# fgcallari/skeres

Hardware: AMD Instinct MI355X
Metric: LM iterations/sec (higher is better)
Workload: dtype f64

## Files before the change

### skeres_amd/csrc/bal_kernels.hip

```cpp
#include <hip/hip_runtime.h>
#include "functors.hpp"
#include "bal_kernels.hpp"

namespace sk {

static constexpr int kBlock = 256;

__device__ __forceinline__ double wave_sum(double v) {
#pragma unroll
  for (int off = 32; off > 0; off >>= 1) v += __shfl_xor(v, off, 64);
  return v;
}

__device__ __forceinline__ int bal_part(const BalDev& d, int i) { return i >= d.cam_b ? 2 : ((i >= d.seg_lo && i < d.cam_a) ? 0 : 1); }
__device__ __forceinline__ int bal_pos(const BalDev& d, int i, int part) { return 9 * (i - (part == 0 ? d.seg_lo : (part == 1 ? d.cam_a : d.cam_b))); }
__device__ __forceinline__ double* bal_block(const BalDev& d, int i, int j, int* ld) {
  const int pj = bal_part(d, j), pi = bal_part(d, i);
  const BalDev::Front& f = d.front[pj];
  const int row = pi == pj ? bal_pos(d, i, pi) : f.border_row[i - d.cam_b];
  *ld = f.ld;
  return f.S + (size_t)row * f.ld + bal_pos(d, j, pj);
}
__device__ __forceinline__ double* bal_rhs(const BalDev& d, int i) {
  const int pi = bal_part(d, i);
// ... 878 lines not shown
}

__global__ __launch_bounds__(256) void tri_pack_kernel(double* S, int ld, double* packed, const int* __restrict__ col0, const long long* __restrict__ off,
                                                       int to_packed) {
  const int kb = blockIdx.y;
  const size_t c0 = (size_t)col0[kb] * 128, width = (size_t)(kb + 1) * 128 - c0;
  double* pk = packed + off[kb];
  const size_t n2 = 128 * width / 2;
  for (size_t i = (size_t)blockIdx.x * 256 + threadIdx.x; i < n2; i += (size_t)gridDim.x * 256) {
    const size_t e = 2 * i, r = e / width, c = e % width;
    double2* a = reinterpret_cast<double2*>(S + ((size_t)kb * 128 + r) * ld + c0 + c);
    double2* b = reinterpret_cast<double2*>(pk + e);
    if (to_packed) *b = *a; else *a = *b;
  }
}

static inline int grid_for(int n, int cap = 2048) {
  int g = (n + kBlock - 1) / kBlock;
  return g < 1 ? 1 : (g > cap ? cap : g);
}

__global__ __launch_bounds__(256) void zero_envelope_kernel(double* S, int ld, const int* col0) {
  const int kb = blockIdx.y;
  const size_t c0 = (size_t)col0[kb] * 128, width = (size_t)(kb + 1) * 128 - c0;
  const size_t n2 = 128 * width / 2;
  for (size_t i = (size_t)blockIdx.x * 256 + threadIdx.x; i < n2; i += (size_t)gridDim.x * 256) {
    const size_t e = 2 * i, r = e / width, c = e % width;
    *reinterpret_cast<double2*>(S + ((size_t)kb * 128 + r) * ld + c0 + c) = make_double2(0.0, 0.0);
  }
}
void launch_zero_envelope(double* S, int ld, const int* col0, int nblk, hipStream_t s) {
  if (nblk > 0) hipLaunchKernelGGL(zero_envelope_kernel, dim3(32, nblk), dim3(256), 0, s, S, ld, col0);
}

int bal_partial_blocks(int N) { return grid_for(N); }
size_t tri_packed_elems(int nblk) { return (size_t)128 * 128 * ((size_t)nblk * (nblk + 1) / 2); }
void launch_tri_pack(double* S, int ld, double* packed, int nblk, const int* col0, const long long* off, bool to_packed, hipStream_t s) {
  if (nblk > 0) hipLaunchKernelGGL(tri_pack_kernel, dim3(64, nblk), dim3(256), 0, s, S, ld, packed, col0, off, to_packed ? 1 : 0);
}

void launch_bal_eval_jac(const BalDev& d, hipStream_t s) {
  if (d.loss_root >= 0) hipLaunchKernelGGL(bal_eval_jac_kernel<true>, dim3(grid_for(d.N)), dim3(kBlock), 0, s, d);
  else hipLaunchKernelGGL(bal_eval_jac_kernel<false>, dim3(grid_for(d.N)), dim3(kBlock), 0, s, d);
}
void launch_bal_eval_cost(const BalDev& d, hipStream_t s) {
  if (d.loss_root >= 0) hipLaunchKernelGGL(bal_eval_cost_kernel<true>, dim3(grid_for(d.N)), dim3(kBlock), 0, s, d);
  else hipLaunchKernelGGL(bal_eval_cost_kernel<false>, dim3(grid_for(d.N)), dim3(kBlock), 0, s, d);
}
int bal_tape_width(const Tape& t) { return t.num_obs_consts > kTapeMaxObs ? 0 : tape_pick_width(t, kBlock); }
template <class K> static void bal_tape_allow_lds(K kernel, size_t bytes) {
  if (bytes > 48 * 1024) (void)hipFuncSetAttribute(reinterpret_cast<const void*>(kernel), hipFuncAttributeMaxDynamicSharedMemorySize, (int)bytes);
}
void launch_bal_eval_jac_tape(const BalDev& d, const TapeDevBuffers& tb, hipStream_t s) {
  const int W = bal_tape_width(tb.host), nobs = tb.host.num_obs_consts;
  const size_t lds = tape_lds_bytes(tb.host, W, kBlock);
  const dim3 g(grid_for(d.N)), b(kBlock);
#define SK_TAPE_JAC(LOSS, WW) { bal_tape_allow_lds(bal_eval_jac_tape_kernel<LOSS, WW>, lds); hipLaunchKernelGGL((bal_eval_jac_tape_kernel<LOSS, WW>), g, b, lds, s, d, tb.view, nobs); }
  if (d.loss_root >= 0) { if (W == 3) SK_TAPE_JAC(true, 3) else if (W == 2) SK_TAPE_JAC(true, 2) else SK_TAPE_JAC(true, 1) }
  else { if (W == 3) SK_TAPE_JAC(false, 3) else if (W == 2) SK_TAPE_JAC(false, 2) else SK_TAPE_JAC(false, 1) }
#undef SK_TAPE_JAC
}
void launch_bal_eval_cost_tape(const BalDev& d, const TapeDevBuffers& tb, hipStream_t s) {
  const size_t lds = tape_lds_bytes(tb.host, 0, kBlock);
  const int nobs = tb.host.num_obs_consts;
  if (d.loss_root >= 0) { bal_tape_allow_lds(bal_eval_cost_tape_kernel<true>, lds); hipLaunchKernelGGL(bal_eval_cost_tape_kernel<true>, dim3(grid_for(d.N)), dim3(kBlock), lds, s, d, tb.view, nobs); }
  else { bal_tape_allow_lds(bal_eval_cost_tape_kernel<false>, lds); hipLaunchKernelGGL(bal_eval_cost_tape_kernel<false>, dim3(grid_for(d.N)), dim3(kBlock), lds, s, d, tb.view, nobs); }
// ... 117 lines not shown
```

### skeres_amd/csrc/bal_kernels.hpp

```cpp
#pragma once
#include <hip/hip_runtime.h>

#include "common.hpp"
#include "loss.hpp"

namespace sk {

constexpr int kLongSegment = 32;
constexpr int kWs = 32;
constexpr int kWu = 28;
struct BalDev {
  int C, P, N;
  int res_size, cam_size, pt_size;
  const int* cam;
  const int* pt;
  const double* obs;
  const int* pt_start;
  const int* cam_start;
  const int* cam_obs;
  int num_segments;
  const int* seg_start;
  const int* seg_row;
  const int* seg_col;
  int num_short_segments, num_long_segments;
// ... 7 lines not shown
  const unsigned char* pseudo;
  const int* kept_home;  const int* kept_global;
  int num_dup;  const int* dup_a;  const int* dup_b;  const int* dup_cam;
  double* xc;  double* xp;
  double* xc_new;  double* xp_new;
  double* scale_c;  double* scale_p;
  double* colsq_c;  double* colsq_p;
  double* gs_c;  double* gs_p;
  double lm_lo, lm_hi, lm_radius;  const double* lm_radius_dev;
  double* step_c;  double* step_p;
  double* y_c;
  double* r;  double* F;  double* E;  double* What;  double* u;
  double* Fcam;  const int* obs_slot;
  double* M;  double* q;
  struct Front { double* S; int ld; int interior; int rhs_row; const int* border_row; };
  Front front[3];
  int seg_lo, cam_a, cam_b;
  const double* y_front[3];
  double* S;  int ld;  int rhs_row;
  double* partial;  int partial_stride;
  int* fail_flag;
  const LossNode* loss_nodes;  int loss_root;  const int* loss_of_obs;
  const unsigned char* is_host;
  int num_host;
  const int* host_obs;
  const double* host_rows;
};
constexpr int kHostRow = 26;
constexpr int kFcam = 20;

int bal_partial_blocks(int N);
int bal_point_blocks(int P);
void launch_zero_envelope(double* S, int ld, const int* col0, int nblk, hipStream_t s);
size_t tri_packed_elems(int nblk);
void launch_tri_pack(double* S, int ld, double* packed, int nblk, const int* col0, const long long* off, bool to_packed, hipStream_t s);
void launch_bal_eval_jac(const BalDev& d, hipStream_t s);
void launch_bal_eval_cost(const BalDev& d, hipStream_t s);
void launch_bal_eval_jac_tape(const BalDev& d, const TapeDevBuffers& tb, hipStream_t s);
void launch_bal_eval_cost_tape(const BalDev& d, const TapeDevBuffers& tb, hipStream_t s);
int launch_bal_host_jac(const BalDev& d, int partial_off, hipStream_t s);
int launch_bal_host_cost(const BalDev& d, int partial_off, hipStream_t s);
void launch_bal_scale_jac(const BalDev& d, hipStream_t s);
void launch_bal_cam_records(const BalDev& d, hipStream_t s);
void launch_bal_reduce(const BalDev& d, hipStream_t s);
void launch_jacobi_scale(const double* colsq, double* scale, int n, hipStream_t s);
void launch_apply_scale_to_reductions(double* colsq, double* gs, const double* scale, int n, hipStream_t s);
void launch_lm_diagonal(const double* colsq, double* D, int n, double lo, double hi, double radius, hipStream_t s);
int launch_grad_max_xnorm(const double* gs, const double* scale, const double* x, int n, double* partial, int stride, hipStream_t s);
void launch_final_reduce(const double* partial, int stride, int count, int K, int maxmask, double* out, hipStream_t s);
void launch_bal_pack_rank_scalars(const double* scal, double* table, int rank, int world, int mode, bool segmented, hipStream_t s);
struct ReduceRows { int n = 0; int row[4] = {0, 0, 0, 0}, count[4] = {0, 0, 0, 0}, is_max[4] = {0, 0, 0, 0}; double* out[4] = {nullptr, nullptr, nullptr, nullptr}; };
void launch_final_reduce_rows(const double* partial, int stride, const ReduceRows& rows, hipStream_t s);
void launch_bal_point_block(const BalDev& d, hipStream_t s);
void launch_bal_kept_points(const BalDev& d, hipStream_t s);
void launch_bal_kept_sums(const BalDev& d, double* buf, int K, bool gather, hipStream_t s);
void launch_bal_obs_precompute(const BalDev& d, hipStream_t s);
void launch_bal_cam_diag(const BalDev& d, hipStream_t s);
void launch_bal_pair(const BalDev& d, hipStream_t s);
void launch_finish_normal_matrix(double* S, int ld, int n, int npad, int rhs_row, const double* D, hipStream_t s);
void launch_bal_finish_S(const BalDev& d, int parts, hipStream_t s);
struct BalFinishRanges { double* S[4] = {nullptr, nullptr, nullptr, nullptr}; int ld[4] = {0, 0, 0, 0}, from[4] = {0, 0, 0, 0}, to[4] = {0, 0, 0, 0}; double value[4] = {0, 0, 0, 0}; };
void launch_bal_finish_all(const BalDev& d, const BalFinishRanges& r, hipStream_t s);
void launch_set_diagonal(double* S, int ld, int from, int to, double value, hipStream_t s);
void launch_bal_backsub(const BalDev& d, double* out, int norm_lo, int norm_hi, int norm_lo2, int norm_hi2, hipStream_t s);

}
// ... 1 lines not shown
```

### skeres_amd/csrc/bal_solver.hip

```cpp
#include <algorithm>
#include <atomic>
#include <map>
#include <thread>
#include <cmath>
#include <limits>
#include <numeric>

#include "bal_kernels.hpp"
#include "bal_plan.hpp"
#include "solver.hpp"

namespace sk {

namespace {

struct CaptureGuard {
  hipStream_t s; bool active; bool* graph_mode;
  CaptureGuard(hipStream_t st, bool on, bool* gm) : s(st), active(on), graph_mode(gm) {}
  void release() { active = false; }
  ~CaptureGuard() {
    if (!active) return;
    hipGraph_t g = nullptr;
    (void)hipStreamEndCapture(s, &g);
    if (g) (void)hipGraphDestroy(g);
// ... 201 lines not shown
  int choose_distribution(const std::vector<int>& opt);
  struct Structure {
    std::vector<int> ocam, opt;
    std::vector<int> band_ocam, band_opt;
    std::vector<int> env_for_model;
    int Creal = 0;
  };
  int init_queues();
  int plan_layout(Structure* st);
  void plan_pack();
  int prepare_pack();
  int shard_or_replicate(const std::vector<int>& opt);
  int cut_camera_sequence(Structure* st);
  void adopt_cuts(const CutPlan& cuts, int Cband, bool multi, Structure* st);
  int upload_structure(const LocalStructure& ls);
  int allocate_fronts(const FrontLayout& lay);
  int bind_device_view(const LocalStructure& ls);
  int agree_with_ranks();
  bool distribution_decided_ = false;
  std::chrono::steady_clock::time_point setup_t0_, stage_last_;
  void stage(const char* what) {
    if (!dev_knobs().debug_setup) return;
    const auto now = std::chrono::steady_clock::now();
    std::fprintf(stderr, "[skeres_amd] set-up: %-40s %8.1f ms (at %.1f ms)\n", what, std::chrono::duration<double, std::milli>(now - stage_last_).count(),
                 std::chrono::duration<double, std::milli>(now - setup_t0_).count());
    stage_last_ = now;
  }
  CholeskyContext chol_ctx_;
  double* h_scal_ = nullptr;
  int partial_stride_ = 0;
  bool zero_by_backsolve_ = false;
  bool need_full_zero_ = false;
  DevBuf<int> b_zero_min_f_[3];
  bool pair_claimed_ = false;
 public:
  ~BalSolver() override {
    if (pair_claimed_) cholesky_release_pair_servers(&chol_ctx_);
    for (hipGraphExec_t g : {g_step_[0], g_step_[1], g_eval_[0], g_eval_[1]}) if (g) (void)hipGraphExecDestroy(g);
    if (h_scal_) (void)hipHostFree(h_scal_);
  }
};

int BalSolver::choose_distribution(const std::vector<int>& opt) {
  const int W = opt_.world;
  distribution_ = SK_DISTRIBUTION_SHARDED;
  if (W <= 1 || opt_.distribution_mode == SK_DISTRIBUTION_SHARDED) return SK_OK;
  if (opt_.distribution_mode != SK_DISTRIBUTION_REPLICATED) {
    const double per_iter = chain_model::shardable_work_s(chain_model::pair_entries(opt, P_total_), (double)opt.size());
    est_saved_s_ = per_iter * (1.0 - 1.0 / W);
    int rc = allreduce(b_pack_.p, packed_elems_);
    if (rc) return rc;
    SK_HIP_TRY(hipStreamSynchronize(stream_));
    const auto t0 = std::chrono::steady_clock::now();
    for (int rep = 0; rep < 2; ++rep) { rc = allreduce(b_pack_.p, packed_elems_); if (rc) return rc; }
    SK_HIP_TRY(hipStreamSynchronize(stream_));
    double mine = std::chrono::duration<double>(std::chrono::steady_clock::now() - t0).count() / 2.0;
    double vals[1] = {mine};
    const int ops[1] = {0};
    SK_HIP_TRY(b_small_.alloc(2 * 9 * (size_t)C_ + 6 * retained_pts_.size() + 64 + 16 * (size_t)W));
    rc = gather_rank_scalars(vals, 1, ops);
    if (rc) return rc;
    est_allreduce_s_ = vals[0] / W;
    collect_allreduce_time(true);
    phase_[5] = 0.0;
    if (est_allreduce_s_ <= est_saved_s_) return SK_OK;
  }
  distribution_ = SK_DISTRIBUTION_REPLICATED;
  opt_.allreduce = nullptr; opt_.world = 1; opt_.rank = 0;
  b_pack_.release();
  return SK_OK;
}

// ... 574 lines not shown
  if (!std::isfinite(cost_)) return SK_ERR_EVALUATION_FAILED;
  return SK_OK;
}

int BalSolver::try_step(double radius, bool* valid, double* mcc, double* new_cost, double* step_norm) {
  bool chain_lost = false;
  int rc = try_step_once(radius, valid, mcc, new_cost, step_norm, &chain_lost);
  if (rc == SK_OK && chain_lost) rc = try_step_once(radius, valid, mcc, new_cost, step_norm, &chain_lost);
  return rc;
}

int BalSolver::try_step_once(double radius, bool* valid, double* mcc, double* new_cost, double* step_norm, bool* chain_lost) {
  hipStream_t s = stream_;
  *chain_lost = false;
  const size_t nc = 9 * (size_t)C_;
  *valid = false;
  SK_HIP_TRY(hipEventRecord(ev_[kEvBegin], s));
  const bool graph = graph_ok();
  const bool replay = graph && g_step_[parity_] != nullptr;
  bool candidate_failed = false;
  if (graph) {
    h_scal_[32] = radius;
    if (!replay && hipStreamBeginCapture(s, hipStreamCaptureModeThreadLocal) != hipSuccess) { (void)hipGetLastError(); graph_mode_ = false; return try_step_once(radius, valid, mcc, new_cost, step_norm, chain_lost); }
  }
  CaptureGuard capture(s, graph && !replay, &graph_mode_);
  if (!replay) {
  d_.lm_lo = opt_.min_lm_diagonal; d_.lm_hi = opt_.max_lm_diagonal; d_.lm_radius = radius; d_.lm_radius_dev = nullptr;
  if (graph) {
    SK_HIP_TRY(hipMemcpyAsync(b_scal_.p + 12, h_scal_ + 32, sizeof(double), hipMemcpyHostToDevice, s));
    d_.lm_radius_dev = b_scal_.p + 12;
  }
  const int bs_resident = opt_.resident_kernels && cholesky_backsolve_resident(npad_ / 128) ? 1 : 0;
  const bool zero_after = zero_by_backsolve_ && bs_resident;
  kt_.begin("memset_S", s);
  for (int f = 0; f < 3; ++f)
    if (fr_[f].nblk > 0) launch_zero_envelope(d_.front[f].S, (int)fr_[f].dim, (zero_by_backsolve_ && !need_full_zero_) ? b_zero_min_f_[f].p : b_zero_col0_f_[f].p, fr_[f].nblk, s);
  kt_.end("memset_S", s);
  need_full_zero_ = !zero_after;
  SK_HIP_TRY(hipMemsetAsync(b_scal_.p + 14, 0, 2 * sizeof(double), s));
  launch_bal_point_block(d_, s);
  launch_bal_kept_points(d_, s);
  launch_bal_obs_precompute(d_, s);
  kt_.begin("bal_cam_diag", s); launch_bal_cam_diag(d_, s); kt_.end("bal_cam_diag", s);
  kt_.begin("bal_pair", s); launch_bal_pair(d_, s); kt_.end("bal_pair", s);
  if (opt_.allreduce && !segmented_) {
    launch_tri_pack(d_.S, npad_, b_pack_.p, npad_ / 128, b_pack_col0_.p, b_pack_off_.p, true, s);
    int rc = allreduce(b_pack_.p, packed_elems_);
    if (rc) return rc;
    launch_tri_pack(d_.S, npad_, b_pack_.p, npad_ / 128, b_pack_col0_.p, b_pack_off_.p, false, s);
  }
  auto finish_root = [&]() {
    launch_bal_finish_S(d_, 4, s);
    launch_set_diagonal(d_.front[2].S, (int)fr_[2].dim, fr_[2].rhs_row, fr_[2].rhs_row + 1, 1e300, s);
    launch_set_diagonal(d_.front[2].S, (int)fr_[2].dim, fr_[2].rhs_row + 1, (int)fr_[2].dim, 1.0, s);
  };
  if (!segmented_) {
    BalFinishRanges r;
    int k = 0;
    for (int f = 0; f < 2; ++f)
      if (fr_[f].nblk > 0 && fr_[f].ncols * 128 > 9 * fr_[f].cams) { r.S[k] = d_.front[f].S; r.ld[k] = (int)fr_[f].dim; r.from[k] = 9 * fr_[f].cams; r.to[k] = fr_[f].ncols * 128; r.value[k] = 1.0; ++k; }
    r.S[k] = d_.front[2].S; r.ld[k] = (int)fr_[2].dim; r.from[k] = fr_[2].rhs_row; r.to[k] = fr_[2].rhs_row + 1; r.value[k] = 1e300; ++k;
    if ((int)fr_[2].dim > fr_[2].rhs_row + 1) { r.S[k] = d_.front[2].S; r.ld[k] = (int)fr_[2].dim; r.from[k] = fr_[2].rhs_row + 1; r.to[k] = (int)fr_[2].dim; r.value[k] = 1.0; ++k; }
    launch_bal_finish_all(d_, r, s);
  } else {
    launch_bal_finish_S(d_, 3, s);
    for (int f = 0; f < 2; ++f)
      if (fr_[f].nblk > 0) launch_set_diagonal(d_.front[f].S, (int)fr_[f].dim, 9 * fr_[f].cams, fr_[f].ncols * 128, 1.0, s);
  }
  if (!graph) SK_HIP_TRY(hipEventRecord(ev_[kEvAssemble], s));
  CholeskyContext* ctx = opt_.lookahead ? &chol_ctx_ : nullptr;
  int* bs_info = bs_resident ? info_p_ : nullptr;
  double* yf[3] = {b_yf_.p + fr_[0].y_off, b_yf_.p + fr_[1].y_off, b_yf_.p + fr_[2].y_off};
  double* wf[3] = {b_wf_.p + fr_[0].y_off, b_wf_.p + fr_[1].y_off, b_wf_.p + fr_[2].y_off};
  const bool prefilled = bs_resident != 0;
  if (prefilled) SK_HIP_TRY(hipMemsetAsync(b_yf_.p, 0xff, (fr_[0].dim + fr_[1].dim + fr_[2].dim) * sizeof(double), s));
  if (segmented_) {
    const FrontView& L = leaf_;
    const FrontHost& R = fr_[2];
    double* Rs = d_.front[2].S;
    double* RLinv = b_Linv_.p + R.linv_off;
    if (L.ncols > 0) {
      cholesky_factor(L.S, L.ld, L.nblk * 128, L.Linv, info_p_, group_, s, ctx, &kt_, L.last, chain_ok(), L.ncols, L.tail_rows, nullptr, L.tail);
      cholesky_border_add(Rs, (long)R.dim, L.S, L.ld, L.ncols, L.nblk - L.ncols, b_leaf_map_.p, s);
    }
    if (replica_) SK_HIP_TRY(hipMemsetAsync(b_pack_.p, 0, packed_elems_ * sizeof(double), s));
    else launch_tri_pack(Rs, (int)R.dim, b_pack_.p, R.nblk, b_pack_col0_.p, b_pack_off_.p, true, s);
    int rc = allreduce(b_pack_.p, packed_elems_);
    if (rc) return rc;
    launch_tri_pack(Rs, (int)R.dim, b_pack_.p, R.nblk, b_pack_col0_.p, b_pack_off_.p, false, s);
    finish_root();
    cholesky_factor(Rs, (long)R.dim, (int)R.dim, RLinv, info_p_, group_, s, ctx, &kt_, R.env(), chain_ok(), -1, 1, nullptr, R.tl());
    cholesky_backsolve(Rs, (long)R.dim, 9 * R.cams, (int)R.dim, R.rhs_row, RLinv, wf[2], yf[2], s, &kt_, R.env(), bs_info, R.tl(), zero_after, bs_resident, prefilled);
    if (L.ncols > 0) {
      cholesky_gather_map(yf[2], b_leaf_gmap_.p, b_ybB_.p, (L.nblk - L.ncols) * 128, s);
      cholesky_backsolve_front(L.S, L.ld, L.nblk, L.ncols, L.rhs_row, L.Linv, b_ybB_.p, wf[0], yf[0], s, L.last, L.spike, L.tail_rows, bs_info, zero_after, L.tail, nullptr, bs_resident, prefilled);
    }
  } else if (dissected_) {
    cholesky_dissected_factor(ds_, info_p_, group_, s, ctx, &chol_ctx_b_, &kt_, &kt_b_, chain_ok());
    cholesky_dissected_backsolve(ds_, 9 * fr_[2].cams, wf[2], yf[2], wf[0], yf[0], wf[1], yf[1], b_ybB_.p, s, &chol_ctx_b_, &kt_, bs_info, zero_after, bs_resident, prefilled);
  } else {
    const FrontHost& R = fr_[2];
    cholesky_factor(d_.front[2].S, (long)R.dim, (int)R.dim, b_Linv_.p, info_p_, group_, s, ctx, &kt_, R.env(), chain_ok(), -1, 1, nullptr, R.tl());
    cholesky_backsolve(d_.front[2].S, (long)R.dim, n_, (int)R.dim, R.rhs_row, b_Linv_.p, wf[2], yf[2], s, &kt_, R.env(), bs_info, R.tl(), zero_after, bs_resident, prefilled);
  }
  if (!graph) SK_HIP_TRY(hipEventRecord(ev_[kEvChol], s));
  {
    int lo = 0, hi = (int)nc, lo2 = 0, hi2 = 0;
    if (segmented_) {
      lo = 9 * my_lo_; hi = 9 * my_hi_;
      if (role_ == 0) { lo2 = 9 * cam_b_; hi2 = (int)nc; }
    }
    launch_bal_backsub(d_, b_scal_.p + 8, lo, hi, lo2, hi2, s);
  }
  if (!graph) SK_HIP_TRY(hipEventRecord(ev_[kEvBacksub], s));
  kt_.begin("bal_eval_cost", s);
  if (tape_mode_) launch_bal_eval_cost_tape(d_, tape_dev_, s); else launch_bal_eval_cost(d_, s);
  kt_.end("bal_eval_cost", s);
  int nb_cost = bal_partial_blocks(N_);
  if (d_.num_host > 0) {
    int rc = host_callbacks(d_.xc_new, false, &candidate_failed);
    if (rc) return rc;
    nb_cost += launch_bal_host_cost(d_, nb_cost, s);
  }
  launch_final_reduce(b_partial_.p, partial_stride_, nb_cost, 2, 0, b_scal_.p, s);
  if (!graph) SK_HIP_TRY(hipEventRecord(ev_[kEvCost], s));
  SK_HIP_TRY(hipMemcpyAsync(h_scal_, b_scal_.p, 16 * sizeof(double), hipMemcpyDeviceToHost, s));
  }
  const bool dev_gather = rank_table_on_device(4) && !graph;
  if (dev_gather) { int rc = enqueue_rank_table(1, 4); if (rc) return rc; }
  if (graph) {
    if (!replay) { capture.release(); int rc = finish_capture(s, &g_step_[parity_]); if (rc) return rc; if (!graph_mode_) return try_step_once(radius, valid, mcc, new_cost, step_norm, chain_lost); }
    SK_HIP_TRY(hipGraphLaunch(g_step_[parity_], s));
    SK_HIP_TRY(hipEventRecord(ev_[kEvCost], s));
  }
  SK_HIP_TRY(hipStreamSynchronize(s));
  float ms = 0.f;
  if (graph) {
    if (hipEventElapsedTime(&ms, ev_[kEvBegin], ev_[kEvCost]) == hipSuccess) phase_[2] += 1e-3 * ms;
  } else {
    if (hipEventElapsedTime(&ms, ev_[kEvBegin], ev_[kEvAssemble]) == hipSuccess) phase_[1] += 1e-3 * ms;
    if (hipEventElapsedTime(&ms, ev_[kEvAssemble], ev_[kEvChol]) == hipSuccess) phase_[2] += 1e-3 * ms;
    if (hipEventElapsedTime(&ms, ev_[kEvChol], ev_[kEvBacksub]) == hipSuccess) phase_[3] += 1e-3 * ms;
    if (hipEventElapsedTime(&ms, ev_[kEvBacksub], ev_[kEvCost]) == hipSuccess) phase_[4] += 1e-3 * ms;
  }
  int fail = 0, info = 0;
  std::memcpy(&fail, h_scal_ + 14, sizeof(int)); std::memcpy(&info, h_scal_ + 15, sizeof(int));
  if (info != 0) need_full_zero_ = true;
  if (cholesky_note_info(opt_.lookahead ? &chol_ctx_ : nullptr, info) && !opt_.allreduce) {
    if (graph_mode_) {
      for (hipGraphExec_t* g : {&g_step_[0], &g_step_[1], &g_eval_[0], &g_eval_[1]}) if (*g) { (void)hipGraphExecDestroy(*g); *g = nullptr; }
      graph_mode_ = false;
    }
    *chain_lost = true;
    return SK_OK;
  }
  double loc[4] = {h_scal_[0], h_scal_[1], h_scal_[9] + (segmented_ ? h_scal_[8] : 0.0), (double)(fail | info)};
  const int ops4[4] = {0, 0, 0, 1};
  int rc = dev_gather ? fold_rank_table(loc, 4, ops4) : gather_rank_scalars(loc, 4, ops4);
  if (rc) return rc;
  if (opt_.allreduce && loc[3] >= 2.0) cholesky_disable_chain(&chol_ctx_);
  const double step_sq = (segmented_ ? 0.0 : h_scal_[8]) + loc[2];
  if (loc[3] != 0.0 || !std::isfinite(step_sq) || !std::isfinite(loc[1])) return SK_OK;
  *valid = true;
  *mcc = -loc[1];
  *new_cost = candidate_failed ? std::numeric_limits<double>::max() : 0.5 * loc[0];
  *step_norm = std::sqrt(step_sq);
  return SK_OK;
}
// ... 90 lines not shown
```

### skeres_amd/csrc/capi.hip

```cpp
#include <cmath>
#include <cstdlib>
#include <new>

#include "bal_kernels.hpp"
#include "dense_kernels.hpp"
#include "dense_rows_kernels.hpp"
#include "solver.hpp"

using namespace sk;

struct sk_ptrvec { std::vector<double*> v; };
struct sk_loss_function { LossFunction l; };
struct sk_cost_function { CostFunction c; };
struct sk_problem { Problem p; };
struct sk_local_parameterization { LocalParameterization p; };
struct sk_options { Options o; };
struct sk_summary { Summary s; };
struct sk_solver { std::unique_ptr<SolverBase> impl; };

static std::string g_program_name;

#define SK_GUARD_BEGIN try {
#define SK_GUARD_END(ret)                                                   \
  } catch (const std::bad_alloc&) { set_error("out of host memory"); return ret; } \
// ... 14 lines not shown
  }
  const int root = (int)loss_nodes.size() - 1;
  loss_root_of.emplace(std::move(key), root);
  has_loss = true;
  return root;
}
}

namespace sk { int rotation_apply(int op, int row_major, int jet_dim, const double* in, int n, double* out); }

namespace sk {
const DevKnobs& dev_knobs() {
  static const DevKnobs knobs = [] {
    DevKnobs k;
    auto num = [](const char* name, int def) { const char* e = getenv(name); return e ? atoi(e) : def; };
    k.chain_server = num("SK_CHOL_CHAIN_SERVER", 1);
    k.bs_resident = num("SK_BS_RESIDENT", 1);
    k.chain_stamps = getenv("SK_CHAIN_STAMPS");
    k.bs_stamps = getenv("SK_BS_STAMPS");
    if (const char* e = getenv("SK_DEBUG")) {
      const std::string topics = std::string(",") + e + ",";
      k.debug_queues = topics.find(",queues,") != std::string::npos;
      k.debug_envelope = topics.find(",envelope,") != std::string::npos;
      k.debug_segments = topics.find(",segments,") != std::string::npos;
      k.debug_setup = topics.find(",setup,") != std::string::npos;
      k.debug_chain_abort = topics.find(",chain_abort,") != std::string::npos;
    }
    k.queue_shift = num("SK_QUEUE_SHIFT", 0);
    k.chain_queues = num("SK_CHAIN_QUEUES", -1);
    k.pair_max_trailing = num("SK_CHAIN_PAIR_MAX_TRAILING", 0);
    k.dissect_at = num("SK_DISSECT_AT", -1);
    k.schedule_plain = num("SK_SCHEDULE_PLAIN", 0);
    k.chain_xcd_local = num("SK_CHAIN_XCD_LOCAL", 0);
    if (const char* e = getenv("SK_BS_PAIR")) k.bs_pair = atoi(e);
    if (const char* e = getenv("SK_BS_SPREAD")) k.bs_spread = atoi(e);
    if (const char* e = getenv("SK_CHAIN_EARLY_SERVER")) k.chain_early_server = atoi(e);
    if (const char* e = getenv("SK_BULK_RESERVE")) {
      k.bulk_reserve = atoi(e);
      const char* c = strchr(e, ',');
      k.bulk_reserve_early = c ? atoi(c + 1) : k.bulk_reserve;
    }
    return k;
  }();
  return knobs;
}
}

extern "C" {

const char* sk_version(void) { return "skeres_amd 0.1 (gfx950)"; }
const char* sk_last_error(void) { return get_error(); }
void sk_init_logging(const char* name) { g_program_name = name ? name : ""; }
int sk_device_count(void) { int n = 0; if (hipGetDeviceCount(&n) != hipSuccess) return 0; return n; }

double* sk_array_new(int n) { if (n < 0) return nullptr; return static_cast<double*>(std::calloc((size_t)(n > 0 ? n : 1), sizeof(double))); }
void sk_array_free(double* a) { std::free(a); }
double sk_array_getitem(const double* a, int i) { return a[i]; }
void sk_array_setitem(double* a, int i, double v) { a[i] = v; }
double* sk_array_slice(double* buffer, int start) { return &buffer[start]; }
void sk_array_copy_in(double* dst, const double* src, int n) { if (n > 0) std::memcpy(dst, src, (size_t)n * sizeof(double)); }
void sk_array_copy_out(const double* src, double* dst, int n) { if (n > 0) std::memcpy(dst, src, (size_t)n * sizeof(double)); }

int sk_matrix_is_null(double* const* m) { return m == nullptr; }
double* sk_matrix_row(double* const* m, int i) { return m[i]; }

sk_ptrvec* sk_ptrvec_new(void) { return new (std::nothrow) sk_ptrvec(); }
// ... 800 lines not shown
  std::memcpy(&FA[((size_t)nA * 128 + msep) * dA], b, (size_t)ra * sizeof(double));
  for (int t1 = 0; t1 < nt; ++t1)
    for (int t2 = 0; t2 <= t1; ++t2) FB[(size_t)t1 * dB + t2] = A[(size_t)(n - 1 - t2) * n + (n - 1 - t1)];
  for (int i = nt; i < nB * 128; ++i) FB[(size_t)i * dB + i] = 1.0;
  for (int k = 0; k < msep; ++k)
    for (int t = 0; t < nt; ++t) FB[((size_t)nB * 128 + k) * dB + t] = A[(size_t)(n - 1 - t) * n + (ra + msep - 1 - k)];
  for (int t = 0; t < nt; ++t) FB[((size_t)nB * 128 + msep) * dB + t] = b[n - 1 - t];
  for (int i = 0; i < msep; ++i) std::memcpy(&FR[(size_t)i * dR], A + (size_t)(ra + i) * n + ra, (size_t)(i + 1) * sizeof(double));
  std::memcpy(&FR[(size_t)msep * dR], b + ra, (size_t)msep * sizeof(double));
  FR[(size_t)msep * dR + msep] = 1e300;
  for (size_t j = (size_t)msep + 1; j < dR; ++j) FR[j * dR + j] = 1.0;
  std::vector<int> mapB(dR, -1);
  for (int k = 0; k < msep; ++k) mapB[k] = msep - 1 - k;
  mapB[msep] = msep;
  const std::vector<int> lastA = host_block_envelope(FA, dA, nA + E), lastB = host_block_envelope(FB, dB, nB + E);
  DevBuf<double> dFA, dFB, dFR, dLinv, dw, dy; DevBuf<int> dinfo, dmap;
  hipStream_t s = nullptr;
  SK_HIP_TRY(dFA.upload(FA, s)); SK_HIP_TRY(dFB.upload(FB, s)); SK_HIP_TRY(dFR.upload(FR, s)); SK_HIP_TRY(dmap.upload(mapB, s));
  SK_HIP_TRY(dLinv.alloc((size_t)(nA + nB + E) * 128 * 128)); SK_HIP_TRY(dLinv.zero(s));
  SK_HIP_TRY(dw.alloc(dA + dB + 2 * dR)); SK_HIP_TRY(dy.alloc(dA + dB + dR)); SK_HIP_TRY(dy.zero(s)); SK_HIP_TRY(dinfo.alloc(1)); SK_HIP_TRY(dinfo.zero(s));
  SK_HIP_TRY(cholesky_init());
  CholeskyContext ctx, ctxB;
  const bool la = ctx.init() == hipSuccess;
  if (!la) (void)hipGetLastError();
  SK_HIP_TRY(hipStreamCreateWithFlags(&s, hipStreamNonBlocking));
  SK_HIP_TRY(hipDeviceSynchronize());
  if (la) cholesky_prepare(&ctx, s);
  const bool side = la && ctxB.init_secondary(ctx) == hipSuccess;
  if (la && !side) (void)hipGetLastError();
  DissectedSystem d;
  d.A.S = dFA.p; d.A.ld = (long)dA; d.A.nblk = nA + E; d.A.ncols = nA; d.A.last = lastA.data(); d.A.Linv = dLinv.p; d.A.rhs_row = nA * 128 + msep;
  d.B.S = dFB.p; d.B.ld = (long)dB; d.B.nblk = nB + E; d.B.ncols = nB; d.B.last = lastB.data(); d.B.Linv = dLinv.p + (size_t)nA * 128 * 128; d.B.rhs_row = nB * 128 + msep;
  d.R.S = dFR.p; d.R.ld = (long)dR; d.R.nblk = E; d.R.ncols = E; d.R.last = nullptr; d.R.Linv = dLinv.p + (size_t)(nA + nB) * 128 * 128; d.R.rhs_row = msep;
  d.border_blocks = E; d.mapB = dmap.p;
  const bool chain = automatic_plan != 0 && la && ctx.server != nullptr;
  cholesky_dissected_factor(d, dinfo.p, group, s, la ? &ctx : nullptr, side ? &ctxB : nullptr, nullptr, nullptr, chain);
  double *wA = dw.p, *wB = dw.p + dA, *wR = dw.p + dA + dB, *ybB = dw.p + dA + dB + dR;
  double *yA = dy.p, *yB = dy.p + dA, *yR = dy.p + dA + dB;
  cholesky_dissected_backsolve(d, msep, wR, yR, wA, yA, wB, yB, ybB, s, side ? &ctxB : nullptr, nullptr, dinfo.p);
  SK_HIP_TRY(hipStreamSynchronize(s));
  SK_HIP_TRY(hipStreamDestroy(s));
  int info = 0;
  SK_HIP_TRY(hipMemcpy(&info, dinfo.p, sizeof(int), hipMemcpyDeviceToHost));
  if (info == 2) { (void)cholesky_note_info(&ctx, info); set_error("the resident panel chain timed out"); return SK_ERR_HIP; }
  if (info) { set_error("matrix is not positive definite"); return SK_ERR_EVALUATION_FAILED; }
  std::vector<double> y(dA + dB + dR);
  SK_HIP_TRY(hipMemcpy(y.data(), dy.p, y.size() * sizeof(double), hipMemcpyDeviceToHost));
  for (int i = 0; i < ra; ++i) x[i] = y[i];
  for (int t = 0; t < nt; ++t) x[n - 1 - t] = y[dA + t];
  for (int k = 0; k < msep; ++k) x[ra + k] = y[dA + dB + k];
  return SK_OK;
  SK_GUARD_END(SK_ERR_INVALID_ARGUMENT)
}

int sk_cholesky_solve_segments(int n, const double* A, const double* b, double* x, int num_segments, const int* cuts, int group, int automatic_plan) {
  SK_GUARD_BEGIN
  const int R = num_segments;
  if (n <= 0 || !A || !b || !x || R < 2 || !cuts) { set_error("invalid argument"); return SK_ERR_INVALID_ARGUMENT; }
  if (sk_device_count() <= 0) { set_error("no HIP device available: libskeres_amd has no CPU fallback"); return SK_ERR_NO_DEVICE; }
  std::vector<int> sb(R + 1, 0), se(R + 1, 0);
  sb[R] = n;
  for (int k = 1; k < R; ++k) { sb[k] = cuts[2 * (k - 1)]; se[k] = cuts[2 * (k - 1) + 1]; }
  for (int k = 1; k <= R; ++k)
    if (sb[k] < se[k - 1] || (k < R && (se[k] < sb[k] || se[k] > n))) { set_error("invalid cuts"); return SK_ERR_INVALID_ARGUMENT; }
  for (int k = 1; k < R; ++k)
    for (int i = se[k]; i < n; ++i)
      for (int j = 0; j < sb[k]; ++j)
// ... 107 lines not shown
```

### skeres_amd/csrc/chol_kernels.hip

```cpp
#include <hip/hip_runtime.h>
#include <algorithm>
#include <atomic>
#include <chrono>
#include <hip/hip_ext.h>
#include <math.h>
#include <stdlib.h>
#include <string.h>
#include <memory>
#include "chol_kernels.hpp"
#include "device_table.hpp"

namespace sk {

typedef double d4 __attribute__((ext_vector_type(4)));

constexpr int gemm_lds_doubles(int kBKT, int kTM, int kTN) { return 2 * (kTM + kTN) * (kBKT + 2); }
#define SK_GEMM_LDS(kBKT, kTM, kTN) __shared__ __attribute__((aligned(16))) double sh[gemm_lds_doubles(kBKT, kTM, kTN)];
template <int kMode, int kShape, int kBKT, int kPF, int kTM, int kTN>
__device__ __forceinline__ void gemm_nt_f64_body(double* shp, double* C, long ldc, const double* A, long lda, const double* B, long ldb, int K,
                                                 int tiles_m, int skip, int main_t = 0x7fffffff, int jump_t = 0, int main_n = 0x7fffffff,
                                                 int jump_n = 0, int block_id = -1, int* first_column_done = nullptr, int count_cols = 1,
                                                 int* diag_done = nullptr) {
  constexpr int mode = kMode;
  constexpr int kLdT = kBKT + 2;
// ... 2295 lines not shown
      env.tail[c] = (unsigned short)(tail ? std::min(std::max(tail[c], 0), nblk - 1) : nblk - tail_rows);
    }
    if (!prefilled) (void)hipMemsetAsync(y, 0xff, sizeof(double) * (size_t)ni, s);
    const bool spread = zero_after && dev_knobs().bs_spread != 0;
    const int janitors = zero_after ? bs_janitors(ncols) : 0;
    hipLaunchKernelGGL(bs_resident_kernel, dim3(spread ? 8 * ncols : ncols + janitors), dim3(1024), 0, s, Linv, S, ld, (const double*)(S + (long)rhs_row * ld), ni, y, nblk, env, info, ncols, yb,
                       spread ? -1 : janitors, yb_map);
    return;
  }
  hipLaunchKernelGGL(copy_row_kernel, dim3((ni + 255) / 256), dim3(256), 0, s, S + (long)rhs_row * ld, w, ni, ni);
  std::vector<int> first(nblk, 0);
  int c0 = 0;
  if (last)
    for (int kb = 0; kb < nblk - 1; ++kb) {
      while (c0 < kb && last[c0] < kb) ++c0;
      first[kb] = c0;
    }
  const int bfirst = first[ncols < nblk - 1 ? ncols : nblk - 1];
  const int bcol0 = (spike || tail) ? 0 : std::min(bfirst, ncols) * 128;
  if (ni > bcol0)
    hipLaunchKernelGGL(bs_border_kernel, dim3((ni - bcol0 + 63) / 64), dim3(1024), 0, s, S + (long)ncols * 128 * ld, ld, m, yb, w, bcol0, ni);
  for (int kb = ncols - 1; kb >= 0; --kb) {
    const int nc = kb * 128, col0 = first[kb] * 128;
    const int grid = nc > col0 ? (nc - col0 + 63) / 64 : 1;
    hipLaunchKernelGGL(bs_step_kernel, dim3(grid), dim3(1024), 0, s, Linv + (long)kb * 128 * 128, S + (long)kb * 128 * ld, ld, w, y, kb, col0, nc);
  }
}

static void fork_join_events(CholeskyContext* c) {
  if (!c->fork_ev) (void)hipEventCreateWithFlags(&c->fork_ev, g_event_flags);
  if (!c->join_ev) (void)hipEventCreateWithFlags(&c->join_ev, g_event_flags);
}

void cholesky_dissected_factor(const DissectedSystem& d, int* info, int group, hipStream_t s, CholeskyContext* ctxA, CholeskyContext* ctxB,
                               KernelTimer* kt, KernelTimer* ktB, bool allow_chain) {
  if (d.A.ncols > 0 && d.B.ncols > 0 && ctxA && ctxB && allow_chain) {
    CholeskyPartner pt{d.B.S, d.B.ld, d.B.nblk, d.B.ncols, 1, d.B.last, d.B.Linv, ctxB, d.B.tail};
    cholesky_factor(d.A.S, d.A.ld, d.A.nblk * 128, d.A.Linv, info, group, s, ctxA, kt, d.A.last, allow_chain, d.A.ncols, 1, &pt, d.A.tail);
    if (!pt.taken)
      cholesky_factor(d.B.S, d.B.ld, d.B.nblk * 128, d.B.Linv, info, group, s, ctxA, kt, d.B.last, allow_chain, d.B.ncols, 1, nullptr, d.B.tail);
    cholesky_border_add(d.R.S, d.R.ld, d.A.S, d.A.ld, d.A.ncols, d.border_blocks, nullptr, s);
    cholesky_border_add(d.R.S, d.R.ld, d.B.S, d.B.ld, d.B.ncols, d.border_blocks, d.mapB, s);
    cholesky_factor(d.R.S, d.R.ld, d.R.nblk * 128, d.R.Linv, info, group, s, ctxA, kt, d.R.last, allow_chain);
    return;
  }
  const bool side = d.B.ncols > 0 && ctxB && ctxB->fork;
  if (d.B.ncols > 0 && !side) {
    cholesky_factor(d.B.S, d.B.ld, d.B.nblk * 128, d.B.Linv, info, group, s, ctxA, kt, d.B.last, allow_chain && ctxB && ctxB->server, d.B.ncols, 1, nullptr, d.B.tail);
  } else if (side) {
    fork_join_events(ctxB);
    hipStream_t sB = ctxB->fork;
    (void)hipEventRecord(ctxB->fork_ev, s);
    (void)hipStreamWaitEvent(sB, ctxB->fork_ev, 0);
    const bool chainB = allow_chain && ctxB->server != nullptr;
    if (!ctxB->runner) ctxB->runner.reset(new AsyncRunner(ctxB->device));
    ctxB->runner->run([&d, info, group, ctxB, ktB, sB, chainB] {
      cholesky_factor(d.B.S, d.B.ld, d.B.nblk * 128, d.B.Linv, info, group, sB, ctxB, ktB, d.B.last, chainB, d.B.ncols, 1, nullptr, d.B.tail);
      (void)hipEventRecord(ctxB->join_ev, sB);
    });
  }
  if (d.A.ncols > 0) cholesky_factor(d.A.S, d.A.ld, d.A.nblk * 128, d.A.Linv, info, group, s, ctxA, kt, d.A.last, allow_chain, d.A.ncols, 1, nullptr, d.A.tail);
  if (side) {
    ctxB->runner->wait();
    (void)hipStreamWaitEvent(s, ctxB->join_ev, 0);
  }
  if (d.A.ncols > 0 && d.B.ncols > 0 && d.mapB && d.mapB_involution) {
    const int m = d.border_blocks * 128;
    hipLaunchKernelGGL(border_add2_kernel, dim3((unsigned)(((long)m * m + 255) / 256)), dim3(256), 0, s, d.R.S, d.R.ld,
                       (const double*)(d.A.S + (long)d.A.ncols * 128 * d.A.ld + (long)d.A.ncols * 128), d.A.ld,
                       (const double*)(d.B.S + (long)d.B.ncols * 128 * d.B.ld + (long)d.B.ncols * 128), d.B.ld, m, d.mapB);
  } else {
    if (d.A.ncols > 0) cholesky_border_add(d.R.S, d.R.ld, d.A.S, d.A.ld, d.A.ncols, d.border_blocks, nullptr, s);
    if (d.B.ncols > 0) cholesky_border_add(d.R.S, d.R.ld, d.B.S, d.B.ld, d.B.ncols, d.border_blocks, d.mapB, s);
  }
  cholesky_factor(d.R.S, d.R.ld, d.R.nblk * 128, d.R.Linv, info, group, s, ctxA, kt, d.R.last, allow_chain);
}

void cholesky_dissected_backsolve(const DissectedSystem& d, int n_root, double* wR, double* yR, double* wA, double* yA, double* wB, double* yB, double* ybB,
                                  hipStream_t s, CholeskyContext* ctxB, KernelTimer* kt, int* info, bool zero_after, int resident, bool prefilled) {
  if (resident < 0) resident = g_bs_resident.load() != 0 ? 1 : 0;
  cholesky_backsolve(d.R.S, d.R.ld, n_root, d.R.nblk * 128, d.R.rhs_row, d.R.Linv, wR, yR, s, nullptr, d.R.last, info, nullptr, zero_after, resident, prefilled);
  if (kt) kt->begin("backsolve", s);
  const int m = d.border_blocks * 128;
  const bool paired = dev_knobs().bs_pair != 0 && d.A.ncols > 0 && d.B.ncols > 0 && info && resident != 0 && d.A.nblk <= kBsPairMaxBlocks && d.B.nblk <= kBsPairMaxBlocks;
  const bool side = !paired && d.B.ncols > 0 && d.A.ncols > 0 && ctxB && ctxB->fork;
  hipStream_t sB = s;
  if (paired) {
    BsPair p;
    const bool spread = zero_after && dev_knobs().bs_spread != 0;
    const FrontView* fv[2] = {&d.A, &d.B};
    double* ys[2] = {yA, yB};
    int grid = 0, jan = 0;
    for (int f = 0; f < 2; ++f) {
      const FrontView& F = *fv[f];
      for (int c = 0; c < F.nblk; ++c) {
        p.env[f].top[c] = (unsigned short)(F.last ? std::min(std::max(F.last[c], c), F.nblk - 1) : F.nblk - 1);
        p.env[f].tail[c] = (unsigned short)(F.tail ? std::min(std::max(F.tail[c], 0), F.nblk - 1) : F.nblk - 1);
      }
      const int janitors = spread ? 3 * F.ncols : (zero_after ? bs_janitors(F.ncols) : 0);
      p.f[f] = BsArgs{F.Linv, F.S, F.ld, (const double*)(F.S + (long)F.rhs_row * F.ld), F.ncols * 128, ys[f], F.nblk, info, F.ncols, yR, janitors, f == 1 ? d.mapB : nullptr,
                      spread ? 3 : 0, spread ? 1 : 0};
      grid += F.ncols; jan += janitors;
    }
    if (spread) { grid = 8 * std::max(d.A.ncols, d.B.ncols); jan = 0; }
    const size_t nA = (size_t)d.A.ncols * 128, nB = (size_t)d.B.ncols * 128;
    if (prefilled) {}
    else if (yB >= yA + nA && (size_t)(yB - yA) <= nA + 4096) (void)hipMemsetAsync(yA, 0xff, sizeof(double) * ((size_t)(yB - yA) + nB), s);
// ... 59 lines not shown
```

### skeres_amd/csrc/dev_knobs.hpp

```cpp
#pragma once

namespace sk {

struct DevKnobs {
  int chain_server = 1;
  int bs_resident = 1;
  const char* chain_stamps = nullptr;
  const char* bs_stamps = nullptr;
  bool debug_queues = false, debug_envelope = false, debug_segments = false, debug_chain_abort = false, debug_setup = false;
  int queue_shift = 0;
  int chain_queues = -1;
  int pair_max_trailing = 0;
  int dissect_at = -1;
  int chain_early_server = 1;
  int bs_spread = 1;
  int bs_pair = 1;
  int bulk_reserve = -1, bulk_reserve_early = -1;
  int chain_xcd_local = 0;
  int schedule_plain = 0;
};
const DevKnobs& dev_knobs();

}
```

Before: 258.6.

## Fuse front zeroing and memsets into one kernel and zero ahead during sync

Replaces the per-front envelope zero launches plus two hipMemsetAsync calls with a single zero_fronts kernel that also clears the flag scalars and 0xff-fills the y buffer. When the backsolve already zeroes the fronts, the next iteration's zeroing is issued right after the step and overlaps the host wait, which now syncs on an event rather than the whole stream. The border_add2 path is also used in the chained dissected factor. The aim is fewer launches and hiding zeroing latency, at the cost of more state-dependent logic around when fronts are valid.

```diff
diff --git a/skeres_amd/csrc/bal_kernels.hip b/skeres_amd/csrc/bal_kernels.hip
--- a/skeres_amd/csrc/bal_kernels.hip
+++ b/skeres_amd/csrc/bal_kernels.hip
@@ -934,6 +934,27 @@
 void launch_zero_envelope(double* S, int ld, const int* col0, int nblk, hipStream_t s) {
   if (nblk > 0) hipLaunchKernelGGL(zero_envelope_kernel, dim3(32, nblk), dim3(256), 0, s, S, ld, col0);
 }
+__global__ __launch_bounds__(256) void zero_fronts_kernel(ZeroFronts z) {
+  int kb = blockIdx.y, f = 0;
+  while (f < 3 && kb >= z.nblk[f]) kb -= z.nblk[f++];
+  if (f == 3) {
+    if (blockIdx.x == 0 && threadIdx.x < 2) z.flags[threadIdx.x] = 0.0;
+    unsigned long long* y = reinterpret_cast<unsigned long long*>(z.fill);
+    for (size_t i = (size_t)blockIdx.x * 256 + threadIdx.x; i < z.fill_n; i += (size_t)gridDim.x * 256) y[i] = ~0ull;
+    return;
+  }
+  double* S = z.S[f];
+  const int ld = z.ld[f];
+  const size_t c0 = (size_t)z.col0[f][kb] * 128, width = (size_t)(kb + 1) * 128 - c0;
+  const size_t n2 = 128 * width / 2;
+  for (size_t i = (size_t)blockIdx.x * 256 + threadIdx.x; i < n2; i += (size_t)gridDim.x * 256) {
+    const size_t e = 2 * i, r = e / width, c = e % width;
+    *reinterpret_cast<double2*>(S + ((size_t)kb * 128 + r) * ld + c0 + c) = make_double2(0.0, 0.0);
+  }
+}
+void launch_zero_fronts(const ZeroFronts& z, hipStream_t s) {
+  hipLaunchKernelGGL(zero_fronts_kernel, dim3(32, z.nblk[0] + z.nblk[1] + z.nblk[2] + 1), dim3(256), 0, s, z);
+}
 
 int bal_partial_blocks(int N) { return grid_for(N); }
 size_t tri_packed_elems(int nblk) { return (size_t)128 * 128 * ((size_t)nblk * (nblk + 1) / 2); }
diff --git a/skeres_amd/csrc/bal_kernels.hpp b/skeres_amd/csrc/bal_kernels.hpp
--- a/skeres_amd/csrc/bal_kernels.hpp
+++ b/skeres_amd/csrc/bal_kernels.hpp
@@ -63,6 +63,9 @@
 int bal_partial_blocks(int N);
 int bal_point_blocks(int P);
 void launch_zero_envelope(double* S, int ld, const int* col0, int nblk, hipStream_t s);
+struct ZeroFronts { double* S[3] = {nullptr, nullptr, nullptr}; int ld[3] = {0, 0, 0}, nblk[3] = {0, 0, 0}; const int* col0[3] = {nullptr, nullptr, nullptr};
+                    double* flags = nullptr; double* fill = nullptr; size_t fill_n = 0; };
+void launch_zero_fronts(const ZeroFronts& z, hipStream_t s);
 size_t tri_packed_elems(int nblk);
 void launch_tri_pack(double* S, int ld, double* packed, int nblk, const int* col0, const long long* off, bool to_packed, hipStream_t s);
 void launch_bal_eval_jac(const BalDev& d, hipStream_t s);
diff --git a/skeres_amd/csrc/bal_solver.hip b/skeres_amd/csrc/bal_solver.hip
--- a/skeres_amd/csrc/bal_solver.hip
+++ b/skeres_amd/csrc/bal_solver.hip
@@ -257,12 +257,23 @@
   bool zero_by_backsolve_ = false;
   bool need_full_zero_ = false;
   DevBuf<int> b_zero_min_f_[3];
+  bool zeroed_ahead_ = false;
+  hipEvent_t ev_scalars_ = nullptr;
+  ZeroFronts zero_fronts(bool full, bool fill) const {
+    ZeroFronts z;
+    for (int f = 0; f < 3; ++f)
+      if (fr_[f].nblk > 0) { z.S[f] = d_.front[f].S; z.ld[f] = (int)fr_[f].dim; z.nblk[f] = fr_[f].nblk; z.col0[f] = full ? b_zero_col0_f_[f].p : b_zero_min_f_[f].p; }
+    z.flags = b_scal_.p + 14;
+    if (fill) { z.fill = b_yf_.p; z.fill_n = fr_[0].dim + fr_[1].dim + fr_[2].dim; }
+    return z;
+  }
   bool pair_claimed_ = false;
  public:
   ~BalSolver() override {
     if (pair_claimed_) cholesky_release_pair_servers(&chol_ctx_);
     for (hipGraphExec_t g : {g_step_[0], g_step_[1], g_eval_[0], g_eval_[1]}) if (g) (void)hipGraphExecDestroy(g);
     if (h_scal_) (void)hipHostFree(h_scal_);
+    if (ev_scalars_) (void)hipEventDestroy(ev_scalars_);
   }
 };
 
@@ -903,12 +914,20 @@
   }
   const int bs_resident = opt_.resident_kernels && cholesky_backsolve_resident(npad_ / 128) ? 1 : 0;
   const bool zero_after = zero_by_backsolve_ && bs_resident;
+  const bool prefilled = bs_resident != 0;
+  const bool one_launch = !graph && !dev_knobs().schedule_plain && dev_knobs().zero_ahead;
+  const bool zeroed_ahead = zeroed_ahead_ && !need_full_zero_ && one_launch;
+  zeroed_ahead_ = false;
   kt_.begin("memset_S", s);
-  for (int f = 0; f < 3; ++f)
-    if (fr_[f].nblk > 0) launch_zero_envelope(d_.front[f].S, (int)fr_[f].dim, (zero_by_backsolve_ && !need_full_zero_) ? b_zero_min_f_[f].p : b_zero_col0_f_[f].p, fr_[f].nblk, s);
+  if (one_launch) {
+    if (!zeroed_ahead) launch_zero_fronts(zero_fronts(!(zero_by_backsolve_ && !need_full_zero_), prefilled), s);
+  } else {
+    for (int f = 0; f < 3; ++f)
+      if (fr_[f].nblk > 0) launch_zero_envelope(d_.front[f].S, (int)fr_[f].dim, (zero_by_backsolve_ && !need_full_zero_) ? b_zero_min_f_[f].p : b_zero_col0_f_[f].p, fr_[f].nblk, s);
+  }
   kt_.end("memset_S", s);
   need_full_zero_ = !zero_after;
-  SK_HIP_TRY(hipMemsetAsync(b_scal_.p + 14, 0, 2 * sizeof(double), s));
+  if (!one_launch) SK_HIP_TRY(hipMemsetAsync(b_scal_.p + 14, 0, 2 * sizeof(double), s));
   launch_bal_point_block(d_, s);
   launch_bal_kept_points(d_, s);
   launch_bal_obs_precompute(d_, s);
@@ -943,8 +962,7 @@
   int* bs_info = bs_resident ? info_p_ : nullptr;
   double* yf[3] = {b_yf_.p + fr_[0].y_off, b_yf_.p + fr_[1].y_off, b_yf_.p + fr_[2].y_off};
   double* wf[3] = {b_wf_.p + fr_[0].y_off, b_wf_.p + fr_[1].y_off, b_wf_.p + fr_[2].y_off};
-  const bool prefilled = bs_resident != 0;
-  if (prefilled) SK_HIP_TRY(hipMemsetAsync(b_yf_.p, 0xff, (fr_[0].dim + fr_[1].dim + fr_[2].dim) * sizeof(double), s));
+  if (prefilled && !one_launch) SK_HIP_TRY(hipMemsetAsync(b_yf_.p, 0xff, (fr_[0].dim + fr_[1].dim + fr_[2].dim) * sizeof(double), s));
   if (segmented_) {
     const FrontView& L = leaf_;
     const FrontHost& R = fr_[2];
@@ -1004,7 +1022,15 @@
     SK_HIP_TRY(hipGraphLaunch(g_step_[parity_], s));
     SK_HIP_TRY(hipEventRecord(ev_[kEvCost], s));
   }
-  SK_HIP_TRY(hipStreamSynchronize(s));
+  if (!graph && !dev_knobs().schedule_plain && dev_knobs().zero_ahead && zero_by_backsolve_ && !need_full_zero_) {
+    if (!ev_scalars_) SK_HIP_TRY(hipEventCreateWithFlags(&ev_scalars_, hipEventDisableTiming));
+    SK_HIP_TRY(hipEventRecord(ev_scalars_, s));
+    launch_zero_fronts(zero_fronts(false, true), s);
+    zeroed_ahead_ = true;
+    SK_HIP_TRY(hipEventSynchronize(ev_scalars_));
+  } else {
+    SK_HIP_TRY(hipStreamSynchronize(s));
+  }
   float ms = 0.f;
   if (graph) {
     if (hipEventElapsedTime(&ms, ev_[kEvBegin], ev_[kEvCost]) == hipSuccess) phase_[2] += 1e-3 * ms;
diff --git a/skeres_amd/csrc/capi.hip b/skeres_amd/csrc/capi.hip
--- a/skeres_amd/csrc/capi.hip
+++ b/skeres_amd/csrc/capi.hip
@@ -70,6 +70,8 @@
     k.dissect_at = num("SK_DISSECT_AT", -1);
     k.schedule_plain = num("SK_SCHEDULE_PLAIN", 0);
     k.chain_xcd_local = num("SK_CHAIN_XCD_LOCAL", 0);
+    k.zero_ahead = num("SK_ZERO_AHEAD", 1);
+    k.border_add2 = num("SK_BORDER_ADD2", 1);
     if (const char* e = getenv("SK_BS_PAIR")) k.bs_pair = atoi(e);
     if (const char* e = getenv("SK_BS_SPREAD")) k.bs_spread = atoi(e);
     if (const char* e = getenv("SK_CHAIN_EARLY_SERVER")) k.chain_early_server = atoi(e);
@@ -936,7 +938,7 @@
   d.A.S = dFA.p; d.A.ld = (long)dA; d.A.nblk = nA + E; d.A.ncols = nA; d.A.last = lastA.data(); d.A.Linv = dLinv.p; d.A.rhs_row = nA * 128 + msep;
   d.B.S = dFB.p; d.B.ld = (long)dB; d.B.nblk = nB + E; d.B.ncols = nB; d.B.last = lastB.data(); d.B.Linv = dLinv.p + (size_t)nA * 128 * 128; d.B.rhs_row = nB * 128 + msep;
   d.R.S = dFR.p; d.R.ld = (long)dR; d.R.nblk = E; d.R.ncols = E; d.R.last = nullptr; d.R.Linv = dLinv.p + (size_t)(nA + nB) * 128 * 128; d.R.rhs_row = msep;
-  d.border_blocks = E; d.mapB = dmap.p;
+  d.border_blocks = E; d.mapB = dmap.p; d.mapB_involution = true;
   const bool chain = automatic_plan != 0 && la && ctx.server != nullptr;
   cholesky_dissected_factor(d, dinfo.p, group, s, la ? &ctx : nullptr, side ? &ctxB : nullptr, nullptr, nullptr, chain);
   double *wA = dw.p, *wB = dw.p + dA, *wR = dw.p + dA + dB, *ybB = dw.p + dA + dB + dR;
diff --git a/skeres_amd/csrc/chol_kernels.hip b/skeres_amd/csrc/chol_kernels.hip
--- a/skeres_amd/csrc/chol_kernels.hip
+++ b/skeres_amd/csrc/chol_kernels.hip
@@ -2351,6 +2351,18 @@
   if (!c->join_ev) (void)hipEventCreateWithFlags(&c->join_ev, g_event_flags);
 }
 
+static void dissected_border_add(const DissectedSystem& d, hipStream_t s) {
+  if (d.A.ncols > 0 && d.B.ncols > 0 && d.mapB && d.mapB_involution && dev_knobs().border_add2) {
+    const int m = d.border_blocks * 128;
+    hipLaunchKernelGGL(border_add2_kernel, dim3((unsigned)(((long)m * m + 255) / 256)), dim3(256), 0, s, d.R.S, d.R.ld,
+                       (const double*)(d.A.S + (long)d.A.ncols * 128 * d.A.ld + (long)d.A.ncols * 128), d.A.ld,
+                       (const double*)(d.B.S + (long)d.B.ncols * 128 * d.B.ld + (long)d.B.ncols * 128), d.B.ld, m, d.mapB);
+  } else {
+    if (d.A.ncols > 0) cholesky_border_add(d.R.S, d.R.ld, d.A.S, d.A.ld, d.A.ncols, d.border_blocks, nullptr, s);
+    if (d.B.ncols > 0) cholesky_border_add(d.R.S, d.R.ld, d.B.S, d.B.ld, d.B.ncols, d.border_blocks, d.mapB, s);
+  }
+}
+
 void cholesky_dissected_factor(const DissectedSystem& d, int* info, int group, hipStream_t s, CholeskyContext* ctxA, CholeskyContext* ctxB,
                                KernelTimer* kt, KernelTimer* ktB, bool allow_chain) {
   if (d.A.ncols > 0 && d.B.ncols > 0 && ctxA && ctxB && allow_chain) {
@@ -2358,8 +2370,7 @@
     cholesky_factor(d.A.S, d.A.ld, d.A.nblk * 128, d.A.Linv, info, group, s, ctxA, kt, d.A.last, allow_chain, d.A.ncols, 1, &pt, d.A.tail);
     if (!pt.taken)
       cholesky_factor(d.B.S, d.B.ld, d.B.nblk * 128, d.B.Linv, info, group, s, ctxA, kt, d.B.last, allow_chain, d.B.ncols, 1, nullptr, d.B.tail);
-    cholesky_border_add(d.R.S, d.R.ld, d.A.S, d.A.ld, d.A.ncols, d.border_blocks, nullptr, s);
-    cholesky_border_add(d.R.S, d.R.ld, d.B.S, d.B.ld, d.B.ncols, d.border_blocks, d.mapB, s);
+    dissected_border_add(d, s);
     cholesky_factor(d.R.S, d.R.ld, d.R.nblk * 128, d.R.Linv, info, group, s, ctxA, kt, d.R.last, allow_chain);
     return;
   }
@@ -2383,15 +2394,7 @@
     ctxB->runner->wait();
     (void)hipStreamWaitEvent(s, ctxB->join_ev, 0);
   }
-  if (d.A.ncols > 0 && d.B.ncols > 0 && d.mapB && d.mapB_involution) {
-    const int m = d.border_blocks * 128;
-    hipLaunchKernelGGL(border_add2_kernel, dim3((unsigned)(((long)m * m + 255) / 256)), dim3(256), 0, s, d.R.S, d.R.ld,
-                       (const double*)(d.A.S + (long)d.A.ncols * 128 * d.A.ld + (long)d.A.ncols * 128), d.A.ld,
-                       (const double*)(d.B.S + (long)d.B.ncols * 128 * d.B.ld + (long)d.B.ncols * 128), d.B.ld, m, d.mapB);
-  } else {
-    if (d.A.ncols > 0) cholesky_border_add(d.R.S, d.R.ld, d.A.S, d.A.ld, d.A.ncols, d.border_blocks, nullptr, s);
-    if (d.B.ncols > 0) cholesky_border_add(d.R.S, d.R.ld, d.B.S, d.B.ld, d.B.ncols, d.border_blocks, d.mapB, s);
-  }
+  dissected_border_add(d, s);
   cholesky_factor(d.R.S, d.R.ld, d.R.nblk * 128, d.R.Linv, info, group, s, ctxA, kt, d.R.last, allow_chain);
 }
 
diff --git a/skeres_amd/csrc/dev_knobs.hpp b/skeres_amd/csrc/dev_knobs.hpp
--- a/skeres_amd/csrc/dev_knobs.hpp
+++ b/skeres_amd/csrc/dev_knobs.hpp
@@ -17,6 +17,8 @@
   int bs_pair = 1;
   int bulk_reserve = -1, bulk_reserve_early = -1;
   int chain_xcd_local = 0;
+  int zero_ahead = 1;
+  int border_add2 = 1;
   int schedule_plain = 0;
 };
 const DevKnobs& dev_knobs();
```

After: 259.5 (median of 4 runs). About the same (+0.3%).
